# lmcinnes/pynndescent

Hardware: AMD Instinct MI355X
Metric: index build: points indexed/sec (recall@10 vs brute force reported alongside) (higher is better)
Workload: dtype f32

## Files before the change

pynndescent_amd/csrc/join.hip:

```cpp
#include "common.h"
#include "metric.h"
#include "gram.h"
#include "state.h"


template <int KS16>
__device__ __forceinline__ bool klist_has(const uint32_t *kl, uint32_t id) {
    uint4 w[KS16 * 4];
#pragma unroll
    for (int c = 0; c < KS16 * 4; c++) w[c] = *(const uint4 *)(kl + 4 * c);
    bool present = false;
#pragma unroll
    for (int c = 0; c < KS16 * 4; c++) present |= (w[c].x == id) | (w[c].y == id) | (w[c].z == id) | (w[c].w == id);
    return present;
}

#ifndef NND_J16_WAVES
#define NND_J16_WAVES 3
#endif
static_assert(NND_CODES_01 == 0 && NND_CODES_0_5 == 1 && NND_CODE_6 == 2, "launch_join_xm and the kernels' names count on these values");
template <int DC, int KS16, bool SHARD, int XM = 0>
__global__ __launch_bounds__(256, NND_J16_WAVES) void k_local_join16(const float *__restrict__ xp, int dp, const float *__restrict__ nrm,
                                                         int metric, const int32_t *__restrict__ cand,
                                                         const int32_t *__restrict__ order, int64_t v_begin,
                                                         int64_t v_end, int k, int ks, const uint32_t *__restrict__ knn_e,
                                                         const float *__restrict__ th, uint64_t *__restrict__ pbuf,
                                                         uint8_t *__restrict__ pdirty, int pcap, uint32_t slot_seed,
                                                         long long *__restrict__ counters, int64_t own_lo, int64_t own_hi,
                                                         uint64_t *__restrict__ pbuf_r, int pcap_r, int64_t rt_lo, int64_t rt_hi) {
    constexpr nnd_metric_family FAM = (nnd_metric_family)XM;
    constexpr int MCP = 16, RV = 32;
    constexpr int NT = DC / 16;
    constexpr int KQ = KS16 * 4;
    constexpr int KQL = RV * KQ / 64;
    constexpr int RPK = 64 / KQ;
    constexpr int kls = KS16 * 16 + 4;
#ifndef NND_J16_QCAP
#define NND_J16_QCAP (8 * 64)
#endif
    constexpr int QCAP = NND_J16_QCAP;
    constexpr int WAVE_BYTES = QCAP * 8 + 2 * RV * 4 + 4 * 4 + 5 * RV * 4 + RV * kls * 4 + 8;
    static_assert((QCAP * 8 + 2 * RV * 4 + 4 * 4 + 5 * RV * 4) % 16 == 0 && (kls * 4) % 16 == 0, "klist must be 16-byte aligned");

    extern __shared__ __attribute__((aligned(16))) unsigned char smem[];
    const int tid = threadIdx.x, lane = nnd_lane(), w = tid >> 6;
    unsigned char *mine = smem + (size_t)w * ((WAVE_BYTES + 15) & ~15);
    uint2 *queue = (uint2 *)mine;
    int32_t *cidbuf = (int32_t *)(queue + QCAP);
    int32_t *nnewbuf = cidbuf + 2 * RV;
    int32_t *cid = nnewbuf + 4;
    float *cnrm = (float *)(cid + RV);
    float *cth = cnrm + RV;
    uint32_t *cslot = (uint32_t *)(cth + RV);
    uint32_t *cflag = cslot + RV;
    uint32_t *klist = cflag + RV;
    const int kq = ks >> 2;
    auto prop_slot = [&](int t, uint32_t slot) __attribute__((always_inline)) -> unsigned long long * {
        if (SHARD && ((int64_t)t < rt_lo || (int64_t)t >= rt_hi))
            return (unsigned long long *)&pbuf_r[(int64_t)t * pcap_r + (slot & (uint32_t)(pcap_r - 1))];
        return (unsigned long long *)&pbuf[(int64_t)t * pcap + slot];
    };
    const int r16 = lane & 15, gq = lane >> 4;
    int64_t n_v = v_end - v_begin;
    int64_t g, stride;
    if ((gridDim.x & 7) == 0) {
        const int64_t per = (((n_v + 7) >> 3) + 3) & ~(int64_t)3;
        const int64_t g0 = (int64_t)(blockIdx.x & 7) * per;
        n_v = n_v < g0 + per ? n_v : g0 + per;
        g = g0 + (int64_t)(blockIdx.x >> 3) * 4 + w;
        stride = (int64_t)(gridDim.x >> 3) * 4;
    } else {
        g = (int64_t)blockIdx.x * 4 + w;
        stride = (int64_t)gridDim.x * 4;
    }

    auto load_cand = [&](int64_t g) __attribute__((always_inline)) -> int {
        const int row = lane < RV ? lane : 0;
        const bool ok = lane < RV && g < n_v;
        const int64_t gg = ok ? g : 0;
        const int64_t v = order ? (int64_t)order[v_begin + gg] : v_begin + gg;
        const int c = cand[v * RV + row];
        return ok ? c : -1;
    };
    auto store_cand = [&](int buf, int c) __attribute__((always_inline)) {
        const unsigned long long m = __ballot(c >= 0 && lane < RV);
        if (lane < RV) cidbuf[buf * RV + lane] = c;
        if (lane == 0) nnewbuf[buf] = __popcll(m & 0xFFFFull) | (__popcll(m >> MCP) << 8);
    };
    f32x4 ra[NT], rb[NT];
    u32x4 klv[KQL];
    float nx_nrm = 0.0f, nx_th = 0.0f;
    int nx_id = -1;
    auto load_rows = [&](const int32_t *cb, int c0, int cw, bool with_old) __attribute__((always_inline)) {
        const int ida = cb[r16], idb = cb[MCP + r16];
        const float *pa = xp + (int64_t)(ida >= 0 ? ida : 0) * dp + c0 + 4 * gq;
        const float *pb = xp + (int64_t)(idb >= 0 ? idb : 0) * dp + c0 + 4 * gq;
#pragma clang loop unroll(full)
        for (int t = 0; t < NT; t++)
            if (16 * t < cw) ra[t] = *(const f32x4 *)(pa + 16 * t);
        if (with_old) {
#pragma clang loop unroll(full)
            for (int t = 0; t < NT; t++)
                if (16 * t < cw) rb[t] = *(const f32x4 *)(pb + 16 * t);
        }
    };
    auto issue_gather = [&](int buf) __attribute__((always_inline)) {
        const int32_t *cb = cidbuf + buf * RV;
        const int cnt = nnewbuf[buf], nn = cnt & 255, no = cnt >> 8;
        if (nn == 0) return;
        load_rows(cb, 0, dp < DC ? dp : DC, no > 0);
        {
            const int row = lane < RV ? lane : 0;
            nx_id = lane < RV ? cb[row] : -1;
            const int64_t ide = nx_id >= 0 ? nx_id : 0;
            nx_nrm = nrm[ide];
            nx_th = th[ide];
#ifdef NND_JOIN_EXTRA_LOAD
            nx_nrm += nrm[(uint32_t)(((uint64_t)(uint32_t)ide * 2654435761ull) % (uint64_t)own_hi)] * 0.0f;
#endif
        }
#pragma clang loop unroll(full)
        for (int i = 0; i < KQL; i++) {
            const int r0 = i * RPK;
            if (!(r0 < MCP ? r0 < nn : r0 - MCP < no)) continue;
            const int idx = lane + i * 64;
            const int r = idx / KQ, c = idx % KQ;
            const int id = cb[r];
            const bool ok = c < kq && id >= 0;
            klv[i] = *(const u32x4 *)(knn_e + (ok ? (int64_t)id * ks + 4 * c : 0));
        }
    };
    auto land_gather = [&](int buf) __attribute__((always_inline)) {
        const int32_t *cb = cidbuf + buf * RV;
        const int cnt = nnewbuf[buf], nn = cnt & 255, no = cnt >> 8;
        if (lane < RV) {
            cid[lane] = nx_id;
            cnrm[lane] = nx_nrm;
            cth[lane] = nx_th;
            cslot[lane] = nnd_hash2(slot_seed, (uint32_t)nx_id) & (uint32_t)(pcap - 1);
            cflag[lane] = 0;
        }
#pragma clang loop unroll(full)
        for (int i = 0; i < KQL; i++) {
            const int r0 = i * RPK;
            if (!(r0 < MCP ? r0 < nn : r0 - MCP < no)) continue;
            const int idx = lane + i * 64;
            const int r = idx / KQ, c = idx % KQ;
            const bool ok = c < kq && cb[r] >= 0 && (int64_t)cb[r] >= own_lo && (int64_t)cb[r] < own_hi;
            const u32x4 empty = {NND_IDX_MASK, NND_IDX_MASK, NND_IDX_MASK, NND_IDX_MASK};
            *(u32x4 *)(klist + r * kls + 4 * c) = ok ? (klv[i] & NND_IDX_MASK) : empty;
        }
    };

    int64_t scan_g = g;
    unsigned long long scan_m = 0;
    int64_t scan_base = g;
    auto next_active = [&]() __attribute__((always_inline)) -> int64_t {
        while (scan_m == 0) {
            if (scan_g >= n_v) return n_v;
            const int64_t gl = scan_g + (int64_t)lane * stride;
            int c0 = -1;
            if (gl < n_v) {
                const int64_t v = order ? (int64_t)order[v_begin + gl] : v_begin + gl;
                c0 = cand[v * RV];
            }
            scan_m = __ballot(c0 >= 0);
            scan_base = scan_g;
            scan_g += 64 * stride;
        }
        const int bit = __builtin_ctzll(scan_m);
        scan_m &= scan_m - 1;
        return scan_base + (int64_t)bit * stride;
    };
    g = next_active();
    int64_t g1 = next_active(), g2 = n_v;
    store_cand(0, load_cand(g));
    store_cand(1, load_cand(g1));
    nnd_wave_lds_sync();
    issue_gather(0);

    int tot_pairs = 0, tot_prop = 0, tot_rows = 0, tot_act = 0, tot_tiles = 0;
    for (int it = 0; g < n_v; g = g1, g1 = g2, it++) {
        g2 = next_active();
        const int cur = it & 1;
        const int my_cnt = nnewbuf[cur], my_new = my_cnt & 255;
        const bool has_old = (my_cnt >> 8) > 0;
        if (my_new > 0) tot_tiles += has_old ? 2 : 1;
        const int c2 = load_cand(g2);
        f32x4 acc[2] = {f32x4{0.f, 0.f, 0.f, 0.f}, f32x4{0.f, 0.f, 0.f, 0.f}};
        if (my_new > 0) {
            land_gather(cur);
            nnd_wave_lds_sync();
            for (int c0 = 0; c0 < dp; c0 += DC) {
                const int cw = (dp - c0) < DC ? (dp - c0) : DC;
                if (c0 > 0) load_rows(cid, c0, cw, has_old);
#ifndef NND_JOIN_NOGRAM
#pragma clang loop unroll(full)
                for (int t = 0; t < NT; t++) {
                    if (16 * t >= cw) continue;
                    if (has_old) {
                        acc[0] = __builtin_amdgcn_mfma_f32_16x16x4f32(ra[t].x, ra[t].x, acc[0], 0, 0, 0);
                        acc[1] = __builtin_amdgcn_mfma_f32_16x16x4f32(ra[t].x, rb[t].x, acc[1], 0, 0, 0);
                        acc[0] = __builtin_amdgcn_mfma_f32_16x16x4f32(ra[t].y, ra[t].y, acc[0], 0, 0, 0);
                        acc[1] = __builtin_amdgcn_mfma_f32_16x16x4f32(ra[t].y, rb[t].y, acc[1], 0, 0, 0);
                        acc[0] = __builtin_amdgcn_mfma_f32_16x16x4f32(ra[t].z, ra[t].z, acc[0], 0, 0, 0);
                        acc[1] = __builtin_amdgcn_mfma_f32_16x16x4f32(ra[t].z, rb[t].z, acc[1], 0, 0, 0);
                        acc[0] = __builtin_amdgcn_mfma_f32_16x16x4f32(ra[t].w, ra[t].w, acc[0], 0, 0, 0);
                        acc[1] = __builtin_amdgcn_mfma_f32_16x16x4f32(ra[t].w, rb[t].w, acc[1], 0, 0, 0);
                    } else {
                        acc[0] = __builtin_amdgcn_mfma_f32_16x16x4f32(ra[t].x, ra[t].x, acc[0], 0, 0, 0);
                        acc[0] = __builtin_amdgcn_mfma_f32_16x16x4f32(ra[t].y, ra[t].y, acc[0], 0, 0, 0);
                        acc[0] = __builtin_amdgcn_mfma_f32_16x16x4f32(ra[t].z, ra[t].z, acc[0], 0, 0, 0);
                        acc[0] = __builtin_amdgcn_mfma_f32_16x16x4f32(ra[t].w, ra[t].w, acc[0], 0, 0, 0);
                    }
                }
#endif
            }
        }
        if (g1 < n_v) issue_gather(cur ^ 1);
        if (my_new > 0) {
            int pid4[4];
            float pn4[4], pth4[4];
#pragma unroll
            for (int r = 0; r < 4; r++) {
                pid4[r] = cid[4 * gq + r];
                pn4[r] = cnrm[4 * gq + r];
                pth4[r] = cth[4 * gq + r];
            }
            int qn = 0;
            auto drain = [&]() __attribute__((always_inline)) {
                nnd_wave_lds_sync();
                for (int base = 0; base < qn; base += 64) {
                    const int t = base + lane;
                    if (t < qn) {
                        const uint2 en = queue[t];
                        const int a = en.x & 31, b = (en.x >> 5) & 31;
                        const float d = __uint_as_float(en.y);
                        const int pid = cid[a], qid = cid[b];
                        if ((en.x & 1024u) && !klist_has<KS16>(klist + a * kls, (uint32_t)qid)) {
#ifndef NND_JOIN_NOATOMIC
                            {
                                unsigned long long *slot = prop_slot(pid, cslot[b]);
                                const unsigned long long key = (unsigned long long)nnd_make_key(d, (uint32_t)qid);
                                atomicMin(slot, key);
                            }
#endif
                            cflag[a] = 1;
                            tot_prop++;
                        }
                        if ((en.x & 2048u) && !klist_has<KS16>(klist + b * kls, (uint32_t)pid)) {
#ifndef NND_JOIN_NOATOMIC
                            {
                                unsigned long long *slot = prop_slot(qid, cslot[a]);
                                const unsigned long long key = (unsigned long long)nnd_make_key(d, (uint32_t)pid);
                                atomicMin(slot, key);
                            }
#endif
                            cflag[b] = 1;
                            tot_prop++;
                        }
                    }
                }
                qn = 0;
            };
#pragma unroll
            for (int J = 0; J < 2; J++) {
                if (J == 1 && !has_old) break;
                if (QCAP < 8 * 64 && J == 1) {
                    drain();
                    nnd_wave_lds_sync();
                }
                const int jj = J * 16 + r16;
                const int qid = cid[jj];
                const float qn_ = cnrm[jj], qth = cth[jj];
#pragma unroll
                for (int r = 0; r < 4; r++) {
                    const int i = 4 * gq + r;
                    const int pid = pid4[r];
                    const bool valid = pid >= 0 && qid >= 0 && (jj >= MCP || jj >= i);
                    tot_pairs += valid ? 1 : 0;
                    const bool self = (pid == qid);
                    const float d = self ? nnd_self_dist<FAM>(metric, pn4[r]) : nnd_gram_to_dist<FAM>(metric, acc[J][r], pn4[r], qn_);
#ifdef NND_JOIN_NOEPI
                    const bool need_p = valid && d == -12345.0f, need_q = false;
#else
                    const bool need_p = valid && d < pth4[r], need_q = valid && !self && d < qth;
#endif
                    const unsigned long long pm = __ballot(need_p | need_q);
                    if (pm) {
                        if (need_p | need_q) {
                            const int off = qn + (int)__builtin_amdgcn_mbcnt_hi((uint32_t)(pm >> 32), __builtin_amdgcn_mbcnt_lo((uint32_t)pm, 0u));
                            queue[off] = make_uint2((uint32_t)i | ((uint32_t)jj << 5) | (need_p ? 1024u : 0u) | (need_q ? 2048u : 0u),
                                                    __float_as_uint(d));
                        }
                        qn += __popcll(pm);
                    }
                }
            }
            drain();
            nnd_wave_lds_sync();
            if (lane < RV && cflag[lane]) pdirty[cid[lane]] = 1;
            if (lane < RV) tot_rows += cid[lane] >= 0;
            if (lane == 0) tot_act += 1;
        }
        nnd_wave_lds_sync();
        store_cand(cur, c2);
    }
    tot_pairs = nnd_wave_sum_i32(tot_pairs);
    tot_prop = nnd_wave_sum_i32(tot_prop);
    tot_rows = nnd_wave_sum_i32(tot_rows);
    tot_act = nnd_wave_sum_i32(tot_act);
    __syncthreads();
    int *red = (int *)smem;
    if (lane == 0) {
        red[w * 5 + 0] = tot_pairs; red[w * 5 + 1] = tot_prop; red[w * 5 + 2] = tot_rows; red[w * 5 + 3] = tot_act;
        red[w * 5 + 4] = tot_tiles;
    }
    __syncthreads();
    if (tid < 5) {
        long long sum = (long long)red[tid] + red[5 + tid] + red[10 + tid] + red[15 + tid];
        if (tid == 4) sum *= (dp >> 2);
        const int which = tid == 0 ? CNT_PAIRS : (tid == 1 ? CNT_PROPOSALS : (tid == 2 ? CNT_ROWS : (tid == 3 ? CNT_ACTIVE : CNT_MFMA)));
        nnd_count(counters, which, sum);
    }
}

static const int32_t *join_order(const nnd_ctx *ctx, int64_t &v_begin, int64_t &v_end) {
    const int32_t *order = nnd_vertex_order(ctx);
    if (!order && ctx->own_order && v_begin >= ctx->own_lo && v_end <= ctx->own_hi) {
        order = ctx->own_order;
        v_begin -= ctx->own_lo;
        v_end -= ctx->own_lo;
    }
    return order;
}

template <int DC, int KS16, bool SHARD, int XM>
static int launch_join16_t(nnd_ctx *ctx, int64_t v_begin, int64_t v_end) {
    constexpr int RV = 32, kls = KS16 * 16 + 4;
    constexpr int WAVE_BYTES = NND_J16_QCAP * 8 + 2 * RV * 4 + 4 * 4 + 5 * RV * 4 + RV * kls * 4 + 8;
    size_t smem = 4 * (size_t)((WAVE_BYTES + 15) & ~15);
    auto kern = k_local_join16<DC, KS16, SHARD, XM>;
    static int wg_per_cu_dev[64] = {0}, n_cu_dev[64] = {0};
    int &wg_per_cu = wg_per_cu_dev[ctx->p.device & 63], &n_cu = n_cu_dev[ctx->p.device & 63];
    if (wg_per_cu == 0) {
        NND_HIP_CHECK(hipFuncSetAttribute((const void *)kern, hipFuncAttributeMaxDynamicSharedMemorySize, (int)smem));
        hipDeviceProp_t prop;
        NND_HIP_CHECK(hipGetDeviceProperties(&prop, ctx->p.device));
        n_cu = prop.multiProcessorCount;
        int occ = 0;
        NND_HIP_CHECK(hipOccupancyMaxActiveBlocksPerMultiprocessor(&occ, (const void *)kern, 256, smem));
        wg_per_cu = occ < 1 ? 1 : occ;
        if (const char *cap = nnd_knob("NND_J16_WGCAP")) {
            const int c = atoi(cap);
            if (c >= 1 && c < wg_per_cu) wg_per_cu = c;
        }
    }
    int64_t nv = v_end - v_begin;
    int64_t groups = (nv + 3) / 4;
    int64_t resident = (int64_t)n_cu * wg_per_cu;
    unsigned grid = (unsigned)(groups < resident ? groups : resident);
    if (grid > 8) grid &= ~7u;
    uint32_t slot_seed = nnd_hash2(ctx->seed ^ 0x2545F491u, (uint32_t)ctx->iter);
    ctx->pbuf_clean = false;
    const int32_t *order = join_order(ctx, v_begin, v_end);
    hipLaunchKernelGGL(kern, dim3(grid), dim3(256), smem, ctx->stream, ctx->xp, ctx->dp, ctx->nrm, ctx->p.metric, ctx->cand,
                       order, v_begin, v_end, ctx->k, ctx->ks, ctx->knn_e, ctx->th, ctx->pbuf, ctx->pdirty, ctx->pcap, slot_seed,
                       ctx->counters, nnd_list_lo(ctx), nnd_list_hi(ctx), ctx->pbuf_r, ctx->pcap_r, ctx->own_lo, ctx->own_hi);
    NND_HIP_CHECK(hipGetLastError());
    return 0;
}

template <int DC, int XM>
static int launch_join16_ks(nnd_ctx *ctx, int64_t v_begin, int64_t v_end) {
    if (ctx->pbuf_r) {
        if (ctx->ks <= 16) return launch_join16_t<DC, 1, true, XM>(ctx, v_begin, v_end);
        if (ctx->ks <= 32) return launch_join16_t<DC, 2, true, XM>(ctx, v_begin, v_end);
        return launch_join16_t<DC, 4, true, XM>(ctx, v_begin, v_end);
    }
    if (ctx->ks <= 16) return launch_join16_t<DC, 1, false, XM>(ctx, v_begin, v_end);
    if (ctx->ks <= 32) return launch_join16_t<DC, 2, false, XM>(ctx, v_begin, v_end);
    return launch_join16_t<DC, 4, false, XM>(ctx, v_begin, v_end);
}

#ifndef NND_JW_WAVES
#define NND_JW_WAVES 3
#endif
#ifndef NND_JW_DCW
#define NND_JW_DCW 16
#endif
#ifndef NND_JW_DC
#define NND_JW_DC 16
#endif
#ifndef NND_JW64_DC
#define NND_JW64_DC 32
#endif
#ifndef NND_JW_WAVES_SPLIT
#define NND_JW_WAVES_SPLIT 4
#endif
#ifndef NND_JW_KL_QCAP
#define NND_JW_KL_QCAP 384
#endif
template <bool KL>
struct join_w_lds {
    static constexpr int QCAP = KL ? NND_JW_KL_QCAP : 512;
    static constexpr int KL_BYTES = KL ? 64 * 128 : 0;
    static constexpr int wave_bytes(int RV) { return KL_BYTES + QCAP * 8 + 2 * RV * 4 + 2 * 4 + 5 * RV * 4 + 8; }
};
__device__ __forceinline__ void nnd_glds16(const void *src, void *lds_dst_wave_uniform) {
    const uint32_t off = __builtin_amdgcn_readfirstlane((uint32_t)(uintptr_t)lds_dst_wave_uniform);
    __builtin_amdgcn_global_load_lds((const __attribute__((address_space(1))) void *)(uintptr_t)src,
                                     (__attribute__((address_space(3))) void *)off, 16, 0, 0);
}
template <int MCP, int DC, bool SHARD, bool BLOCKED = false, bool SKIP_TRI = false, int ASEL = -1, bool KL = false, int XM = 0>
__global__ __launch_bounds__(256, MCP == 32 ? (ASEL >= 0 ? NND_JW_WAVES_SPLIT : NND_JW_WAVES) : 2) void k_local_join_w(const float *__restrict__ xp, int dp,
                                                                       const float *__restrict__ nrm, int metric,
                                                                       const int32_t *__restrict__ cand,
                                                                       const int32_t *__restrict__ order, int64_t v_begin,
                                                                       int64_t v_end, int k, int ks,
                                                                       const uint32_t *__restrict__ knn_e,
                                                                       const float *__restrict__ th, uint64_t *__restrict__ pbuf,
                                                                       uint8_t *__restrict__ pdirty, int pcap, uint32_t slot_seed,
                                                                       long long *__restrict__ counters, int64_t own_lo, int64_t own_hi,
                                                                       uint64_t *__restrict__ pbuf_r, int pcap_r, int64_t rt_lo, int64_t rt_hi,
                                                                       int cstride, int new_off, int old_off) {
    static_assert(!BLOCKED || MCP == 64, "the blocked passes run the 64-slot kernel");
    constexpr nnd_metric_family FAM = (nnd_metric_family)XM;
    constexpr int NA = MCP / 16, NB = 2 * NA, RV = 2 * MCP;
    constexpr int NT = DC / 16;
    constexpr int RPL = RV / 64;
    static_assert(!KL || (MCP == 32 && !SHARD && !BLOCKED && ASEL < 0), "staged neighbour lists: the plain 32-slot kernel only");
    constexpr int QCAP = join_w_lds<KL>::QCAP;
    constexpr int WAVE_BYTES = join_w_lds<KL>::wave_bytes(RV);

    extern __shared__ __attribute__((aligned(16))) unsigned char smem[];
    const int tid = threadIdx.x, lane = nnd_lane(), w = tid >> 6;
    unsigned char *mine = smem + (size_t)w * ((WAVE_BYTES + 15) & ~15);
    uint32_t *klist = (uint32_t *)mine;
    uint2 *queue = (uint2 *)(mine + join_w_lds<KL>::KL_BYTES);
    int32_t *cidbuf = (int32_t *)(queue + QCAP);
    int32_t *nnewbuf = cidbuf + 2 * RV;
    int32_t *cid = nnewbuf + 2;
    float *cnrm = (float *)(cid + RV);
    float *cth = cnrm + RV;
    uint32_t *cslot = (uint32_t *)(cth + RV);
    uint32_t *cflag = cslot + RV;
    const int kq = ks >> 2;
    auto prop_slot = [&](int t, uint32_t slot) __attribute__((always_inline)) -> unsigned long long * {
        if (SHARD && ((int64_t)t < rt_lo || (int64_t)t >= rt_hi))
            return (unsigned long long *)&pbuf_r[(int64_t)t * pcap_r + (slot & (uint32_t)(pcap_r - 1))];
        return (unsigned long long *)&pbuf[(int64_t)t * pcap + slot];
    };
    const int r16 = lane & 15, gq = lane >> 4;
    int64_t n_v = v_end - v_begin;
    int64_t g, stride;
    if ((gridDim.x & 7) == 0) {
        const int64_t per = (((n_v + 7) >> 3) + 3) & ~(int64_t)3;
        const int64_t g0 = (int64_t)(blockIdx.x & 7) * per;
        n_v = n_v < g0 + per ? n_v : g0 + per;
        g = g0 + (int64_t)(blockIdx.x >> 3) * 4 + w;
        stride = (int64_t)(gridDim.x >> 3) * 4;
    } else {
        g = (int64_t)blockIdx.x * 4 + w;
        stride = (int64_t)gridDim.x * 4;
    }

    auto load_cand = [&](int64_t g, int (&c)[RPL]) __attribute__((always_inline)) {
        const bool ok = g < n_v;
        const int64_t gg = ok ? g : 0;
        const int64_t v = order ? (int64_t)order[v_begin + gg] : v_begin + gg;
#pragma unroll
        for (int u = 0; u < RPL; u++) {
            const int cc = BLOCKED ? cand[v * cstride + (u == 0 ? new_off : old_off) + lane] : cand[v * RV + lane + 64 * u];
            c[u] = ok ? cc : -1;
        }
    };
    auto store_cand = [&](int buf, const int (&c)[RPL]) __attribute__((always_inline)) {
        int nn = 0, no = 0;
#pragma unroll
        for (int u = 0; u < RPL; u++) {
            const unsigned long long m = __ballot(c[u] >= 0);
            cidbuf[buf * RV + lane + 64 * u] = c[u];
            if (RPL == 1) {
                nn += __popcll(m & 0xFFFFFFFFull);
                no += __popcll(m >> 32);
            } else {
                if (u == 0) nn += __popcll(m); else no += __popcll(m);
            }
        }
        if (lane == 0) nnewbuf[buf] = nn | (no << 8);
    };
    f32x4 rt[NB][NT];
    f32x4 rt2[NB][NT];
    float nx_nrm[RPL], nx_th[RPL];
    int nx_id[RPL];
    auto tile_live = [&](int t, int nn, int no) __attribute__((always_inline)) -> bool {
        return t < NA ? 16 * t < nn : 16 * (t - NA) < no;
    };
    constexpr int A_LO = ASEL >= 0 ? ASEL : 0;
    constexpr int NEW_MIN = 16 * A_LO;
    auto tile_needed = [&](int t) __attribute__((always_inline)) -> bool {
        return ASEL < 0 || t == ASEL || t >= (SKIP_TRI ? NA : ASEL);
    };
    auto load_rows_into = [&](f32x4 (&dst)[NB][NT], const int32_t *cb, int c0, int cw, int nn, int no) __attribute__((always_inline)) {
#pragma unroll
        for (int t = 0; t < NB; t++) {
            if (!tile_needed(t) || !tile_live(t, nn, no)) continue;
            const int id = cb[16 * t + r16];
            const float *pr = xp + (int64_t)(id >= 0 ? id : 0) * dp + c0 + 4 * gq;
#pragma unroll
            for (int j = 0; j < NT; j++)
                if (16 * j < cw) dst[t][j] = *(const f32x4 *)(pr + 16 * j);
        }
    };
    auto load_rows = [&](const int32_t *cb, int c0, int cw, int nn, int no) __attribute__((always_inline)) { load_rows_into(rt, cb, c0, cw, nn, no); };
    auto issue_gather = [&](int buf) __attribute__((always_inline)) {
        const int32_t *cb = cidbuf + buf * RV;
        const int cnt = nnewbuf[buf], nn = cnt & 255, no = cnt >> 8;
        if (nn <= NEW_MIN) return;
        load_rows(cb, 0, dp < DC ? dp : DC, nn, no);
#pragma unroll
        for (int u = 0; u < RPL; u++) {
            nx_id[u] = cb[lane + 64 * u];
            const int64_t ide = nx_id[u] >= 0 ? nx_id[u] : 0;
            nx_nrm[u] = nrm[ide];
            nx_th[u] = th[ide];
        }
    };
    auto land_gather = [&]() __attribute__((always_inline)) {
#pragma unroll
        for (int u = 0; u < RPL; u++) {
            const int r = lane + 64 * u;
            cid[r] = nx_id[u];
            cnrm[r] = nx_nrm[u];
            cth[r] = nx_th[u];
            cslot[r] = nnd_hash2(slot_seed, (uint32_t)nx_id[u]) & (uint32_t)(pcap - 1);
            cflag[r] = 0;
        }
    };
    auto list_has = [&](int row, uint32_t id) __attribute__((always_inline)) -> bool {
        if ((int64_t)row < own_lo || (int64_t)row >= own_hi) return false;
        const u32x4 *kl = (const u32x4 *)(knn_e + (int64_t)row * ks);
        bool present = false;
        for (int c = 0; c < kq; c += 4) {
            u32x4 wv[4];
#pragma unroll
            for (int j = 0; j < 4; j++) wv[j] = kl[c + j < kq ? c + j : c];
#pragma unroll
            for (int j = 0; j < 4; j++) {
                const u32x4 m = wv[j] & NND_IDX_MASK;
                present |= (c + j < kq) && ((m.x == id) | (m.y == id) | (m.z == id) | (m.w == id));
            }
        }
        return present;
    };
    auto issue_lists = [&](int nn, int no) __attribute__((always_inline)) {
#pragma unroll 1
        for (int i = 0; i < 8; i++) {
            if (!(8 * i < MCP ? 8 * i < nn : 8 * i - MCP < no)) continue;
            const int row = 8 * i + (lane >> 3), c = lane & 7;
            const int id = cid[row];
            if (id >= 0 && c < kq) nnd_glds16(knn_e + (int64_t)id * ks + 4 * c, klist + i * 256);
        }
    };
    auto list_has_lds = [&](int row, uint32_t id) __attribute__((always_inline)) -> bool {
        const u32x4 *kl = (const u32x4 *)(klist + row * 32);
        bool present = false;
        for (int h = 0; h < kq; h += 4) {
            u32x4 wv[4];
#pragma unroll
            for (int j = 0; j < 4; j++) wv[j] = kl[h + ((j + row) & 3)];
#pragma unroll
            for (int j = 0; j < 4; j++) {
                const u32x4 m = wv[j] & NND_IDX_MASK;
                present |= (m.x == id) | (m.y == id) | (m.z == id) | (m.w == id);
            }
        }
        return present;
    };
    int tot_pairs = 0, tot_prop = 0, tot_rows = 0, tot_act = 0, tot_tiles = 0;
    int qn = 0;
    auto drain = [&]() __attribute__((always_inline)) {
        nnd_wave_lds_sync();
        for (int base = 0; base < qn; base += 64) {
            const int t = base + lane;
            if (t < qn) {
                const uint2 en = queue[t];
                const int a = en.x & 63, b = (en.x >> 6) & 127;
                const float d = __uint_as_float(en.y);
                const int pid = cid[a], qid = cid[b];
                if ((en.x & (1u << 13)) && !(KL ? list_has_lds(a, (uint32_t)qid) : list_has(pid, (uint32_t)qid))) {
                    atomicMin(prop_slot(pid, cslot[b]), (unsigned long long)nnd_make_key(d, (uint32_t)qid));
                    cflag[a] = 1;
                    tot_prop++;
                }
                if ((en.x & (1u << 14)) && !(KL ? list_has_lds(b, (uint32_t)pid) : list_has(qid, (uint32_t)pid))) {
                    atomicMin(prop_slot(qid, cslot[a]), (unsigned long long)nnd_make_key(d, (uint32_t)pid));
                    cflag[b] = 1;
                    tot_prop++;
                }
            }
        }
        nnd_wave_lds_sync();
        qn = 0;
    };

    {
        int c0[RPL], c1[RPL];
        load_cand(g, c0);
        load_cand(g + stride, c1);
        store_cand(0, c0);
        store_cand(1, c1);
    }
    nnd_wave_lds_sync();
    issue_gather(0);

    for (int it = 0; g < n_v; g += stride, it++) {
        const int cur = it & 1;
        const int my_cnt = nnewbuf[cur], nn = my_cnt & 255, no = my_cnt >> 8;
        int c2[RPL];
        load_cand(g + 2 * stride, c2);
        f32x4 acc[NA][NB];
#pragma unroll
        for (int a = 0; a < NA; a++)
#pragma unroll
            for (int b = 0; b < NB; b++) acc[a][b] = f32x4{0.f, 0.f, 0.f, 0.f};
        if (nn > NEW_MIN) {
            land_gather();
            nnd_wave_lds_sync();
            if constexpr (KL) issue_lists(nn, no);
            auto gram_block = [&](const f32x4 (&r)[NB][NT], int c0, int cw) __attribute__((always_inline)) {
#pragma unroll
                for (int a = 0; a < NA; a++) {
                    if ((ASEL >= 0 && a != ASEL) || !tile_live(a, nn, no)) continue;
#pragma unroll
                    for (int b = SKIP_TRI ? NA : a; b < NB; b++) {
                        if (!tile_live(b, nn, no)) continue;
                        if (c0 == 0) tot_tiles++;
#pragma unroll
                        for (int j = 0; j < NT; j++) {
                            if (16 * j >= cw) continue;
                            acc[a][b] = __builtin_amdgcn_mfma_f32_16x16x4f32(r[a][j].x, r[b][j].x, acc[a][b], 0, 0, 0);
                            acc[a][b] = __builtin_amdgcn_mfma_f32_16x16x4f32(r[a][j].y, r[b][j].y, acc[a][b], 0, 0, 0);
                            acc[a][b] = __builtin_amdgcn_mfma_f32_16x16x4f32(r[a][j].z, r[b][j].z, acc[a][b], 0, 0, 0);
                            acc[a][b] = __builtin_amdgcn_mfma_f32_16x16x4f32(r[a][j].w, r[b][j].w, acc[a][b], 0, 0, 0);
                        }
                    }
                }
            };
            for (int c0 = 0; c0 < dp; c0 += 2 * DC) {
                const int cw = (dp - c0) < DC ? (dp - c0) : DC;
                const int c1 = c0 + DC, cw1 = (dp - c1) < DC ? (dp - c1) : DC;
#ifndef NND_JW_NO_PIPELINE
                if constexpr (ASEL >= 0) {
                    if (c0 > 0) load_rows_into(rt, cid, c0, cw, nn, no);
                    gram_block(rt, c0, cw);
                    if (c1 < dp) {
                        load_rows_into(rt, cid, c1, cw1, nn, no);
                        gram_block(rt, c1, cw1);
                    }
                    continue;
                }
                if (c1 < dp) load_rows_into(rt2, cid, c1, cw1, nn, no);
                gram_block(rt, c0, cw);
                if (c1 < dp) {
                    if (c1 + DC < dp) load_rows_into(rt, cid, c1 + DC, (dp - c1 - DC) < DC ? (dp - c1 - DC) : DC, nn, no);
                    gram_block(rt2, c1, cw1);
                }
#else
                gram_block(rt, c0, cw);
                if (c1 < dp) {
                    load_rows_into(rt2, cid, c1, cw1, nn, no);
                    gram_block(rt2, c1, cw1);
                    if (c1 + DC < dp) load_rows_into(rt, cid, c1 + DC, (dp - c1 - DC) < DC ? (dp - c1 - DC) : DC, nn, no);
                }
#endif
            }
        }
        if constexpr (KL) {
            if (nn > NEW_MIN) asm volatile("s_waitcnt vmcnt(0)" ::: "memory");
        }
        if (g + stride < n_v) issue_gather(cur ^ 1);
        if (nn > NEW_MIN) {
#pragma unroll
            for (int a = 0; a < NA; a++) {
                if ((ASEL >= 0 && a != ASEL) || !tile_live(a, nn, no)) continue;
                int pid4[4];
                float pn4[4], pth4[4];
#pragma unroll
                for (int r = 0; r < 4; r++) {
                    pid4[r] = cid[16 * a + 4 * gq + r];
                    pn4[r] = cnrm[16 * a + 4 * gq + r];
                    pth4[r] = cth[16 * a + 4 * gq + r];
                }
#pragma unroll
                for (int b = SKIP_TRI ? NA : a; b < NB; b++) {
                    if (!tile_live(b, nn, no)) continue;
                    const int jj = 16 * b + r16;
                    const int qid = cid[jj];
                    const float qn_ = cnrm[jj], qth = cth[jj];
#pragma unroll
                    for (int r = 0; r < 4; r++) {
                        const int i = 16 * a + 4 * gq + r;
                        const int pid = pid4[r];
                        const bool valid = pid >= 0 && qid >= 0 && (jj >= MCP || jj >= i);
                        tot_pairs += valid ? 1 : 0;
                        const bool self = (pid == qid);
                        const float d = self ? nnd_self_dist<FAM>(metric, pn4[r]) : nnd_gram_to_dist<FAM>(metric, acc[a][b][r], pn4[r], qn_);
                        const bool need_p = valid && d < pth4[r], need_q = valid && !self && d < qth;
                        const unsigned long long pm = __ballot(need_p | need_q);
                        if (pm) {
                            if (need_p | need_q) {
                                const int off = qn + (int)__builtin_amdgcn_mbcnt_hi((uint32_t)(pm >> 32), __builtin_amdgcn_mbcnt_lo((uint32_t)pm, 0u));
                                queue[off] = make_uint2((uint32_t)i | ((uint32_t)jj << 6) | (need_p ? (1u << 13) : 0u) | (need_q ? (1u << 14) : 0u),
                                                        __float_as_uint(d));
                            }
                            qn += __popcll(pm);
                        }
                    }
                    if (qn > QCAP - 256) drain();
                }
            }
            if (qn > 0) drain();
            nnd_wave_lds_sync();
#pragma unroll
            for (int u = 0; u < RPL; u++) {
                const int r = lane + 64 * u;
                if (cflag[r]) pdirty[cid[r]] = 1;
                if (ASEL <= 0) tot_rows += cid[r] >= 0;
            }
            if (ASEL <= 0 && lane == 0) tot_act += 1;
        }
        nnd_wave_lds_sync();
        store_cand(cur, c2);
    }
    tot_pairs = nnd_wave_sum_i32(tot_pairs);
    tot_prop = nnd_wave_sum_i32(tot_prop);
    tot_rows = nnd_wave_sum_i32(tot_rows);
    tot_act = nnd_wave_sum_i32(tot_act);
    __syncthreads();
    int *red = (int *)smem;
    if (lane == 0) {
        red[w * 5 + 0] = tot_pairs; red[w * 5 + 1] = tot_prop; red[w * 5 + 2] = tot_rows; red[w * 5 + 3] = tot_act;
        red[w * 5 + 4] = tot_tiles;
    }
    __syncthreads();
    if (tid < 5) {
        long long sum = (long long)red[tid] + red[5 + tid] + red[10 + tid] + red[15 + tid];
        if (tid == 4) sum *= (dp >> 2);
        const int which = tid == 0 ? CNT_PAIRS : (tid == 1 ? CNT_PROPOSALS : (tid == 2 ? CNT_ROWS : (tid == 3 ? CNT_ACTIVE : CNT_MFMA)));
        nnd_count(counters, which, sum);
    }
}

template <int MCP, int DC, bool SHARD, bool BLOCKED, bool SKIP_TRI, int ASEL, bool KL, int XM>
static int launch_join_w_t(nnd_ctx *ctx, int64_t v_begin, int64_t v_end, int cstride = 0, int new_off = 0, int old_off = 0) {
    constexpr int RV = 2 * MCP;
    constexpr int WAVE_BYTES = join_w_lds<KL>::wave_bytes(RV);
    size_t smem = 4 * (size_t)((WAVE_BYTES + 15) & ~15);
    auto kern = k_local_join_w<MCP, DC, SHARD, BLOCKED, SKIP_TRI, ASEL, KL, XM>;
    static int wg_per_cu_dev[64] = {0}, n_cu_dev[64] = {0};
    int &wg_per_cu = wg_per_cu_dev[ctx->p.device & 63], &n_cu = n_cu_dev[ctx->p.device & 63];
    if (wg_per_cu == 0) {
        NND_HIP_CHECK(hipFuncSetAttribute((const void *)kern, hipFuncAttributeMaxDynamicSharedMemorySize, (int)smem));
        hipDeviceProp_t prop;
        NND_HIP_CHECK(hipGetDeviceProperties(&prop, ctx->p.device));
        n_cu = prop.multiProcessorCount;
        int occ = 0;
        NND_HIP_CHECK(hipOccupancyMaxActiveBlocksPerMultiprocessor(&occ, (const void *)kern, 256, smem));
        wg_per_cu = occ < 1 ? 1 : occ;
    }
    int64_t nv = v_end - v_begin;
    int64_t groups = (nv + 3) / 4;
    int64_t resident = (int64_t)n_cu * wg_per_cu;
    unsigned grid = (unsigned)(groups < resident ? groups : resident);
    if (grid > 8) grid &= ~7u;
    uint32_t slot_seed = nnd_hash2(ctx->seed ^ 0x2545F491u, (uint32_t)ctx->iter);
    ctx->pbuf_clean = false;
    const int32_t *order = join_order(ctx, v_begin, v_end);
    hipLaunchKernelGGL(kern, dim3(grid), dim3(256), smem, ctx->stream, ctx->xp, ctx->dp, ctx->nrm, ctx->p.metric, ctx->cand,
                       order, v_begin, v_end, ctx->k, ctx->ks, ctx->knn_e, ctx->th, ctx->pbuf, ctx->pdirty,
                       ctx->pcap, slot_seed, ctx->counters, nnd_list_lo(ctx), nnd_list_hi(ctx), ctx->pbuf_r, ctx->pcap_r, ctx->own_lo, ctx->own_hi,
                       cstride, new_off, old_off);
    NND_HIP_CHECK(hipGetLastError());
    return 0;
}

template <int MCP, int DC, int XM>
static int launch_join_w(nnd_ctx *ctx, int64_t v_begin, int64_t v_end) {
#ifdef NND_JW_SPLIT
    if (MCP == 32) {
        if (ctx->pbuf_r) {
            if (launch_join_w_t<MCP, DC, true, false, false, 0, false, XM>(ctx, v_begin, v_end)) return 1;
            return launch_join_w_t<MCP, DC, true, false, false, 1, false, XM>(ctx, v_begin, v_end);
        }
        if (launch_join_w_t<MCP, DC, false, false, false, 0, false, XM>(ctx, v_begin, v_end)) return 1;
        return launch_join_w_t<MCP, DC, false, false, false, 1, false, XM>(ctx, v_begin, v_end);
    }
#endif
#ifndef NND_JW_NO_LDS_LISTS
    if constexpr (MCP == 32) {
        if (!ctx->pbuf_r && ctx->ks <= 32 && nnd_list_lo(ctx) <= 0 && nnd_list_hi(ctx) >= ctx->n && !(ctx->p.flags & NND_FLAG_TEST_JOIN_UNSTAGED)) {
            static int kl_ok_dev[64] = {0};
            int &kl_ok = kl_ok_dev[ctx->p.device & 63];
            if (kl_ok == 0) {
                constexpr size_t smem = 4 * (size_t)((join_w_lds<true>::wave_bytes(2 * MCP) + 15) & ~15);
                auto kern = k_local_join_w<MCP, DC, false, false, false, -1, true, XM>;
                int occ = 0;
                if (hipFuncSetAttribute((const void *)kern, hipFuncAttributeMaxDynamicSharedMemorySize, (int)smem) != hipSuccess ||
                    hipOccupancyMaxActiveBlocksPerMultiprocessor(&occ, (const void *)kern, 256, smem) != hipSuccess) {
                    (void)hipGetLastError();
                    occ = 0;
                }
                kl_ok = occ >= 3 ? 1 : -1;
            }
            if (kl_ok > 0) return launch_join_w_t<MCP, DC, false, false, false, -1, true, XM>(ctx, v_begin, v_end);
        }
    }
#endif
    return ctx->pbuf_r ? launch_join_w_t<MCP, DC, true, false, false, -1, false, XM>(ctx, v_begin, v_end)
                        : launch_join_w_t<MCP, DC, false, false, false, -1, false, XM>(ctx, v_begin, v_end);
}

template <bool SHARD, int XM>
static int launch_join_blocked(nnd_ctx *ctx, int64_t v_begin, int64_t v_end) {
    if (launch_join_w_t<64, 32, SHARD, true, false, -1, false, XM>(ctx, v_begin, v_end, 256, 0, 128)) return 1;
    if (launch_join_w_t<64, 32, SHARD, true, true, -1, false, XM>(ctx, v_begin, v_end, 256, 0, 192)) return 1;
    if (launch_join_w_t<64, 32, SHARD, true, false, -1, false, XM>(ctx, v_begin, v_end, 256, 64, 128)) return 1;
    if (launch_join_w_t<64, 32, SHARD, true, true, -1, false, XM>(ctx, v_begin, v_end, 256, 64, 192)) return 1;
    return launch_join_w_t<64, 32, SHARD, true, true, -1, false, XM>(ctx, v_begin, v_end, 256, 0, 64);
}

template <int XM>
static int launch_join_xm(nnd_ctx *ctx, int64_t v_begin, int64_t v_end) {
    const bool wide = ctx->dp >= 128;
    switch (ctx->mcp) {
#ifndef NND_J16_DCW
#define NND_J16_DCW 64
#endif
        case 16: return wide ? launch_join16_ks<NND_J16_DCW, XM>(ctx, v_begin, v_end) : launch_join16_ks<32, XM>(ctx, v_begin, v_end);
        case 32: return wide ? launch_join_w<32, NND_JW_DCW, XM>(ctx, v_begin, v_end) : launch_join_w<32, NND_JW_DC, XM>(ctx, v_begin, v_end);
        case 64: return launch_join_w<64, NND_JW64_DC, XM>(ctx, v_begin, v_end);
        case 128: return ctx->pbuf_r ? launch_join_blocked<true, XM>(ctx, v_begin, v_end) : launch_join_blocked<false, XM>(ctx, v_begin, v_end);
    }
    ctx->set_error("unsupported padded max_candidates %d", ctx->mcp);
    return 1;
}

int nnd_launch_join(nnd_ctx *ctx, int64_t v_begin, int64_t v_end) {
    if (v_end <= v_begin) return 0;
    if (ctx->p.metric == 6) return launch_join_xm<NND_CODE_6>(ctx, v_begin, v_end);
    return ctx->p.metric >= 2 ? launch_join_xm<NND_CODES_0_5>(ctx, v_begin, v_end) : launch_join_xm<NND_CODES_01>(ctx, v_begin, v_end);
}
```

Baseline: 54.70 million.

## Deepen candidate prefetch and screen join distances before queueing proposals

Candidate loading now runs one vertex further ahead: the order lookup and candidate reads are prefetched and the new/old counts are kept in registers rather than read back from LDS. The epilogue first computes every pair distance with the metric specialised at compile time, and ballots whether any pair beats a threshold, so the queue and drain path can be skipped when nothing qualifies. Validity checks are folded into -INF thresholds for missing candidates, and the pair, row and active counters are computed arithmetically on the scalar side without wave reductions. This adds pipeline state, more live registers and extra LDS syncs, and the counter arithmetic must still match the old per-lane validity logic.

Result: no change. 54.99 million, median of 6 (+0.5%).

```diff
diff --git a/pynndescent_amd/csrc/join.hip b/pynndescent_amd/csrc/join.hip
--- a/pynndescent_amd/csrc/join.hip
+++ b/pynndescent_amd/csrc/join.hip
@@ -2,7 +2,14 @@
 #include "metric.h"
 #include "gram.h"
 #include "state.h"
-
+#include <type_traits>
+
+typedef int32_t i32x4 __attribute__((ext_vector_type(4)));
+
+__device__ __forceinline__ int nnd_opaque_sgpr(int v) {
+    asm volatile("" : "+s"(v));
+    return v;
+}
 
 template <int KS16>
 __device__ __forceinline__ bool klist_has(const uint32_t *kl, uint32_t id) {
@@ -43,7 +50,7 @@
     static_assert((QCAP * 8 + 2 * RV * 4 + 4 * 4 + 5 * RV * 4) % 16 == 0 && (kls * 4) % 16 == 0, "klist must be 16-byte aligned");
 
     extern __shared__ __attribute__((aligned(16))) unsigned char smem[];
-    const int tid = threadIdx.x, lane = nnd_lane(), w = tid >> 6;
+    const int tid = threadIdx.x, lane = nnd_lane(), w = __builtin_amdgcn_readfirstlane(tid >> 6);
     unsigned char *mine = smem + (size_t)w * ((WAVE_BYTES + 15) & ~15);
     uint2 *queue = (uint2 *)mine;
     int32_t *cidbuf = (int32_t *)(queue + QCAP);
@@ -74,24 +81,26 @@
         stride = (int64_t)gridDim.x * 4;
     }
 
-    auto load_cand = [&](int64_t g) __attribute__((always_inline)) -> int {
+    auto vertex_at = [&](int64_t g) __attribute__((always_inline)) -> int64_t {
+        const int64_t gg = g < n_v ? g : 0;
+        return order ? (int64_t)order[v_begin + gg] : v_begin + gg;
+    };
+    auto load_cand = [&](int64_t g, int64_t v) __attribute__((always_inline)) -> int {
         const int row = lane < RV ? lane : 0;
-        const bool ok = lane < RV && g < n_v;
-        const int64_t gg = ok ? g : 0;
-        const int64_t v = order ? (int64_t)order[v_begin + gg] : v_begin + gg;
         const int c = cand[v * RV + row];
-        return ok ? c : -1;
-    };
-    auto store_cand = [&](int buf, int c) __attribute__((always_inline)) {
+        return lane < RV && g < n_v ? c : -1;
+    };
+    auto store_cand = [&](int buf, int c) __attribute__((always_inline)) -> int {
         const unsigned long long m = __ballot(c >= 0 && lane < RV);
         if (lane < RV) cidbuf[buf * RV + lane] = c;
-        if (lane == 0) nnewbuf[buf] = __popcll(m & 0xFFFFull) | (__popcll(m >> MCP) << 8);
+        return __popcll(m & 0xFFFFull) | (__popcll(m >> MCP) << 8);
     };
     f32x4 ra[NT], rb[NT];
     u32x4 klv[KQL];
     float nx_nrm = 0.0f, nx_th = 0.0f;
     int nx_id = -1;
     auto load_rows = [&](const int32_t *cb, int c0, int cw, bool with_old) __attribute__((always_inline)) {
+        cw = nnd_opaque_sgpr(cw);
         const int ida = cb[r16], idb = cb[MCP + r16];
         const float *pa = xp + (int64_t)(ida >= 0 ? ida : 0) * dp + c0 + 4 * gq;
         const float *pb = xp + (int64_t)(idb >= 0 ? idb : 0) * dp + c0 + 4 * gq;
@@ -104,9 +113,9 @@
                 if (16 * t < cw) rb[t] = *(const f32x4 *)(pb + 16 * t);
         }
     };
-    auto issue_gather = [&](int buf) __attribute__((always_inline)) {
+    auto issue_gather = [&](int buf, int cnt) __attribute__((always_inline)) {
         const int32_t *cb = cidbuf + buf * RV;
-        const int cnt = nnewbuf[buf], nn = cnt & 255, no = cnt >> 8;
+        const int nn = cnt & 255, no = cnt >> 8;
         if (nn == 0) return;
         load_rows(cb, 0, dp < DC ? dp : DC, no > 0);
         {
@@ -130,13 +139,13 @@
             klv[i] = *(const u32x4 *)(knn_e + (ok ? (int64_t)id * ks + 4 * c : 0));
         }
     };
-    auto land_gather = [&](int buf) __attribute__((always_inline)) {
+    auto land_gather = [&](int buf, int cnt) __attribute__((always_inline)) {
         const int32_t *cb = cidbuf + buf * RV;
-        const int cnt = nnewbuf[buf], nn = cnt & 255, no = cnt >> 8;
+        const int nn = cnt & 255, no = cnt >> 8;
         if (lane < RV) {
             cid[lane] = nx_id;
             cnrm[lane] = nx_nrm;
-            cth[lane] = nx_th;
+            cth[lane] = nx_id >= 0 ? nx_th : -INFINITY;
             cslot[lane] = nnd_hash2(slot_seed, (uint32_t)nx_id) & (uint32_t)(pcap - 1);
             cflag[lane] = 0;
         }
@@ -173,26 +182,29 @@
         return scan_base + (int64_t)bit * stride;
     };
     g = next_active();
-    int64_t g1 = next_active(), g2 = n_v;
-    store_cand(0, load_cand(g));
-    store_cand(1, load_cand(g1));
+    int64_t g1 = next_active(), g2 = next_active(), g3 = n_v;
+    int my_cnt = store_cand(0, load_cand(g, vertex_at(g)));
+    int c_next = load_cand(g1, vertex_at(g1));
+    int64_t v2 = vertex_at(g2);
     nnd_wave_lds_sync();
-    issue_gather(0);
+    issue_gather(0, my_cnt);
 
     int tot_pairs = 0, tot_prop = 0, tot_rows = 0, tot_act = 0, tot_tiles = 0;
-    for (int it = 0; g < n_v; g = g1, g1 = g2, it++) {
-        g2 = next_active();
+    for (int it = 0; g < n_v; g = g1, g1 = g2, g2 = g3, it++) {
+        g3 = next_active();
         const int cur = it & 1;
-        const int my_cnt = nnewbuf[cur], my_new = my_cnt & 255;
-        const bool has_old = (my_cnt >> 8) > 0;
+        const int my_new = my_cnt & 255, my_old = my_cnt >> 8;
+        const bool has_old = my_old > 0;
         if (my_new > 0) tot_tiles += has_old ? 2 : 1;
-        const int c2 = load_cand(g2);
         f32x4 acc[2] = {f32x4{0.f, 0.f, 0.f, 0.f}, f32x4{0.f, 0.f, 0.f, 0.f}};
         if (my_new > 0) {
-            land_gather(cur);
+            land_gather(cur, my_cnt);
             nnd_wave_lds_sync();
+        }
+        const int64_t v3 = vertex_at(g3);
+        if (my_new > 0) {
             for (int c0 = 0; c0 < dp; c0 += DC) {
-                const int cw = (dp - c0) < DC ? (dp - c0) : DC;
+                const int cw = nnd_opaque_sgpr((dp - c0) < DC ? (dp - c0) : DC);
                 if (c0 > 0) load_rows(cid, c0, cw, has_old);
 #ifndef NND_JOIN_NOGRAM
 #pragma clang loop unroll(full)
@@ -217,15 +229,53 @@
 #endif
             }
         }
-        if (g1 < n_v) issue_gather(cur ^ 1);
+        const int nx_cnt = store_cand(cur ^ 1, c_next);
+        nnd_wave_lds_sync();
+        c_next = load_cand(g2, v2);
+        v2 = v3;
+        if (g1 < n_v) issue_gather(cur ^ 1, nx_cnt);
         if (my_new > 0) {
             int pid4[4];
             float pn4[4], pth4[4];
-#pragma unroll
-            for (int r = 0; r < 4; r++) {
-                pid4[r] = cid[4 * gq + r];
-                pn4[r] = cnrm[4 * gq + r];
-                pth4[r] = cth[4 * gq + r];
+            {
+                const i32x4 pi = *(const i32x4 *)(cid + 4 * gq);
+                const f32x4 pn = *(const f32x4 *)(cnrm + 4 * gq), pt = *(const f32x4 *)(cth + 4 * gq);
+#pragma unroll
+                for (int r = 0; r < 4; r++) {
+                    pid4[r] = pi[r];
+                    pn4[r] = pn[r];
+                    pth4[r] = pt[r];
+                }
+            }
+            tot_pairs += (my_new * (my_new + 1) >> 1) + my_new * my_old;
+            tot_rows += my_new + my_old;
+            tot_act += 1;
+            unsigned long long any = 0;
+            auto screen = [&](auto code) __attribute__((always_inline)) {
+                const int mc = decltype(code)::value >= 0 ? decltype(code)::value : metric;
+#pragma unroll
+                for (int J = 0; J < 2; J++) {
+                    if (J == 1 && !has_old) break;
+                    const int jj = J * 16 + r16;
+                    const int qid = cid[jj];
+                    const float qn_ = cnrm[jj], qth = cth[jj];
+#pragma unroll
+                    for (int r = 0; r < 4; r++) {
+                        const float dg = nnd_gram_to_dist<FAM>(mc, acc[J][r], pn4[r], qn_), ds = nnd_self_dist<FAM>(mc, pn4[r]);
+                        const float d = pid4[r] == qid ? ds : dg;
+                        acc[J][r] = d;
+#ifndef NND_JOIN_NOEPI
+                        any |= __builtin_amdgcn_ballot_w64((d < pth4[r]) | (d < qth));
+#endif
+                    }
+                    __builtin_amdgcn_sched_barrier(0);
+                }
+            };
+            if constexpr (FAM == NND_CODES_01) {
+                if (metric == 0) screen(std::integral_constant<int, 0>{});
+                else screen(std::integral_constant<int, 1>{});
+            } else {
+                screen(std::integral_constant<int, -1>{});
             }
             int qn = 0;
             auto drain = [&]() __attribute__((always_inline)) {
@@ -263,53 +313,44 @@
                 }
                 qn = 0;
             };
-#pragma unroll
-            for (int J = 0; J < 2; J++) {
-                if (J == 1 && !has_old) break;
-                if (QCAP < 8 * 64 && J == 1) {
-                    drain();
-                    nnd_wave_lds_sync();
-                }
-                const int jj = J * 16 + r16;
-                const int qid = cid[jj];
-                const float qn_ = cnrm[jj], qth = cth[jj];
-#pragma unroll
-                for (int r = 0; r < 4; r++) {
-                    const int i = 4 * gq + r;
-                    const int pid = pid4[r];
-                    const bool valid = pid >= 0 && qid >= 0 && (jj >= MCP || jj >= i);
-                    tot_pairs += valid ? 1 : 0;
-                    const bool self = (pid == qid);
-                    const float d = self ? nnd_self_dist<FAM>(metric, pn4[r]) : nnd_gram_to_dist<FAM>(metric, acc[J][r], pn4[r], qn_);
-#ifdef NND_JOIN_NOEPI
-                    const bool need_p = valid && d == -12345.0f, need_q = false;
-#else
-                    const bool need_p = valid && d < pth4[r], need_q = valid && !self && d < qth;
-#endif
-                    const unsigned long long pm = __ballot(need_p | need_q);
-                    if (pm) {
-                        if (need_p | need_q) {
-                            const int off = qn + (int)__builtin_amdgcn_mbcnt_hi((uint32_t)(pm >> 32), __builtin_amdgcn_mbcnt_lo((uint32_t)pm, 0u));
-                            queue[off] = make_uint2((uint32_t)i | ((uint32_t)jj << 5) | (need_p ? 1024u : 0u) | (need_q ? 2048u : 0u),
-                                                    __float_as_uint(d));
+            if (any) {
+#pragma unroll
+                for (int J = 0; J < 2; J++) {
+                    if (J == 1 && !has_old) break;
+                    if (QCAP < 8 * 64 && J == 1) {
+                        drain();
+                        nnd_wave_lds_sync();
+                    }
+                    const int jj = J * 16 + r16;
+                    const int qid = cid[jj];
+                    const float qth = cth[jj];
+#pragma unroll
+                    for (int r = 0; r < 4; r++) {
+                        const int i = 4 * gq + r;
+                        const int pid = pid4[r];
+                        const float d = acc[J][r];
+                        const bool tri = jj >= MCP || jj >= i;
+                        const bool need_p = tri && qid >= 0 && d < pth4[r], need_q = tri && pid >= 0 && pid != qid && d < qth;
+                        const unsigned long long pm = __builtin_amdgcn_ballot_w64(need_p | need_q);
+                        if (pm) {
+                            if (need_p | need_q) {
+                                const int off = qn + (int)__builtin_amdgcn_mbcnt_hi((uint32_t)(pm >> 32), __builtin_amdgcn_mbcnt_lo((uint32_t)pm, 0u));
+                                queue[off] = make_uint2((uint32_t)i | ((uint32_t)jj << 5) | (need_p ? 1024u : 0u) | (need_q ? 2048u : 0u),
+                                                        __float_as_uint(d));
+                            }
+                            qn += __popcll(pm);
                         }
-                        qn += __popcll(pm);
                     }
                 }
-            }
-            drain();
-            nnd_wave_lds_sync();
-            if (lane < RV && cflag[lane]) pdirty[cid[lane]] = 1;
-            if (lane < RV) tot_rows += cid[lane] >= 0;
-            if (lane == 0) tot_act += 1;
+                drain();
+                nnd_wave_lds_sync();
+                if (lane < RV && cflag[lane]) pdirty[cid[lane]] = 1;
+            }
         }
         nnd_wave_lds_sync();
-        store_cand(cur, c2);
-    }
-    tot_pairs = nnd_wave_sum_i32(tot_pairs);
+        my_cnt = nx_cnt;
+    }
     tot_prop = nnd_wave_sum_i32(tot_prop);
-    tot_rows = nnd_wave_sum_i32(tot_rows);
-    tot_act = nnd_wave_sum_i32(tot_act);
     __syncthreads();
     int *red = (int *)smem;
     if (lane == 0) {
```
